# FalkorDB/FalkorDB

Hardware: NVIDIA B200
Metric: traversed edges/sec (mxm TEPS), 3-hop ANY_PAIR mxm chain (higher is better)
Workload: dtype bool/u32 index

## Files before the change

### falkordb_b200/csrc/bits.cu

```cuda
#include "common.cuh"
#include "ops.cuh"
#include <cub/block/block_reduce.cuh>
#include <algorithm>
#include <cstring>

namespace b200 {

template <int W> struct PullCfg {
    static constexpr int WL = W >= 4 ? 4 : W;
    static constexpr int SPLIT = W / WL;
    static constexpr int VG = 8 / SPLIT;
};
static const u64 PUSH_CHUNK = 8192;
static const u64 LONG_ROW = 4096;
static const u64 LONG_CHUNK = 8192;

static void require_natural(const DevBits &X, const char *what);

u32 bits_words_for(u64 nrows) {
    if (nrows == 0) return 1;
    u64 w = (nrows + 63) / 64;
    if (w > 16) return 0;
    u32 p = 1;
    while (p < w) p <<= 1;
    return p;
}

__global__ void k_bits_scatter(const u64 *__restrict__ Ap, const u32 *__restrict__ Aj, u64 nrows, u64 nnz,
                               u64 *__restrict__ X, u32 W) {
    u64 q = (u64)blockIdx.x * blockDim.x + threadIdx.x;
    u64 stride = (u64)gridDim.x * blockDim.x;
    for (; q < nnz; q += stride) {
        u64 lo = 0, hi = nrows - 1;
        while (lo < hi) {
            u64 mid = (lo + hi + 1) >> 1;
            if (Ap[mid] <= q) lo = mid; else hi = mid - 1;
        }
        u32 col = Aj[q];
        atomicOr((unsigned long long *)&X[(u64)col * W + (lo >> 6)], 1ULL << (lo & 63));
    }
}

void bits_from_csr(const DevCSR &F, DevBits &X) {
    u32 W = bits_words_for(F.nrows);
    if (!W) throw GrbError(-8, "bit-frontier form needs <= 1024 rows");
    X.clear();
    X.nrows = F.nrows; X.ncols = F.ncols; X.W = W;
    X.w.alloc(F.ncols * W);
    X.w.zero();
    if (F.nnz)
        LAUNCH(k_bits_scatter, grid_for(F.nnz, 256, 1 << 16), 256, 0, F.p.ptr, F.j.ptr, F.nrows, F.nnz, X.w.ptr, W);
}

static const u32 TILE_V = 1024;
static const u32 TILE_THREADS = 512;

__device__ __forceinline__ u32 transpose32(u32 x, u32 lane) {
    u32 y;
    y = __shfl_xor_sync(0xffffffffu, x, 16);
    x = (lane & 16) ? ((x & 0xFFFF0000u) | ((y & 0xFFFF0000u) >> 16)) : ((x & 0x0000FFFFu) | ((y & 0x0000FFFFu) << 16));
    y = __shfl_xor_sync(0xffffffffu, x, 8);
    x = (lane & 8) ? ((x & 0xFF00FF00u) | ((y & 0xFF00FF00u) >> 8)) : ((x & 0x00FF00FFu) | ((y & 0x00FF00FFu) << 8));
    y = __shfl_xor_sync(0xffffffffu, x, 4);
    x = (lane & 4) ? ((x & 0xF0F0F0F0u) | ((y & 0xF0F0F0F0u) >> 4)) : ((x & 0x0F0F0F0Fu) | ((y & 0x0F0F0F0Fu) << 4));
    y = __shfl_xor_sync(0xffffffffu, x, 2);
    x = (lane & 2) ? ((x & 0xCCCCCCCCu) | ((y & 0xCCCCCCCCu) >> 2)) : ((x & 0x33333333u) | ((y & 0x33333333u) << 2));
    y = __shfl_xor_sync(0xffffffffu, x, 1);
    x = (lane & 1) ? ((x & 0xAAAAAAAAu) | ((y & 0xAAAAAAAAu) >> 1)) : ((x & 0x55555555u) | ((y & 0x55555555u) << 1));
    return x;
}

__global__ void __launch_bounds__(TILE_THREADS)
k_bits_count(const u64 *__restrict__ X, u64 n, u32 W, u64 ntiles, u32 *__restrict__ tc) {
    __shared__ u32 wc[TILE_THREADS / 32][64];
    const u32 tid = threadIdx.x, warp = tid >> 5, lane = tid & 31;
    u64 tile = blockIdx.x;
    u64 v0 = tile * TILE_V + (u64)warp * 64;
    for (u32 w = 0; w < W; w++) {
        u32 clo = 0, chi = 0;
#pragma unroll
        for (u32 g = 0; g < 2; g++) {
            u64 v = v0 + g * 32 + lane;
            u64 word = (v < n) ? X[v * W + w] : 0ULL;
            if (__ballot_sync(0xffffffffu, word != 0ULL)) {
                clo += __popc(transpose32((u32)word, lane));
                chi += __popc(transpose32((u32)(word >> 32), lane));
            }
        }
        wc[warp][lane] = clo;
        wc[warp][lane + 32] = chi;
        __syncthreads();
        if (tid < 64) {
            u32 s = 0;
#pragma unroll
            for (u32 q = 0; q < TILE_THREADS / 32; q++) s += wc[q][tid];
            tc[((u64)w * 64 + tid) * ntiles + tile] = s;
        }
        __syncthreads();
    }
}

__device__ __forceinline__ void csa(u64 &hi, u64 &lo, u64 a, u64 b, u64 c) {
    const u64 u = a ^ b;
    hi = (a & b) | (u & c);
    lo = u ^ c;
}
template <int WL> __device__ __forceinline__ void ld_part(u64 (&x)[WL], const u64 *p) {
    if constexpr (WL == 1) { x[0] = __ldg(p); }
    else if constexpr (WL == 2) { ulonglong2 v = __ldg(reinterpret_cast<const ulonglong2 *>(p)); x[0] = v.x; x[1] = v.y; }
    else { u64x4 v = ld_v4(p); x[0] = v.a; x[1] = v.b; x[2] = v.c; x[3] = v.d; }
}
template <int W>
__global__ void __launch_bounds__(128)
k_bits_count_csa(const u64 *__restrict__ X, u64 n, u64 ntiles, u32 *__restrict__ tc) {
    constexpr int WL = PullCfg<W>::WL, SPLIT = PullCfg<W>::SPLIT;
    const u32 lane = threadIdx.x & 31;
    const u64 wid = ((u64)blockIdx.x * blockDim.x + threadIdx.x) >> 5;
    const u64 tile = wid / SPLIT;
    const u32 h = (u32)(wid % SPLIT);
    if (tile >= ntiles) return;
    const u64 vbase = tile * TILE_V;
    u64 plane[6][WL];
    u64 pend[5][WL];
#pragma unroll
    for (int p = 0; p < 6; p++)
#pragma unroll
        for (int w = 0; w < WL; w++) plane[p][w] = 0;
#pragma unroll
    for (int i = 0; i < 16; i++) {
        u64 xa[WL], xb[WL];
        const u64 va = vbase + lane + 64 * (u64)i, vb_ = va + 32;
        if (va < n) ld_part<WL>(xa, X + va * W + h * WL); else { for (int w = 0; w < WL; w++) xa[w] = 0; }
        if (vb_ < n) ld_part<WL>(xb, X + vb_ * W + h * WL); else { for (int w = 0; w < WL; w++) xb[w] = 0; }
#pragma unroll
        for (int w = 0; w < WL; w++) {
            u64 c;
            csa(c, plane[0][w], plane[0][w], xa[w], xb[w]);
#pragma unroll
            for (int L = 1; L < 6; L++) {
                if ((i >> (L - 1)) & 1) {
                    if (L < 5) { u64 c2; csa(c2, plane[L][w], plane[L][w], pend[L - 1][w], c); c = c2; }
                    else plane[5][w] ^= 0;
                } else { pend[L - 1][w] = c; break; }
            }
            if (i == 15) plane[5][w] = c;
        }
    }
#pragma unroll
    for (int w = 0; w < WL; w++) {
        u32 clo = 0, chi = 0;
#pragma unroll
        for (int p = 0; p < 6; p++) {
            clo += __popc(transpose32((u32)plane[p][w], lane)) << p;
            chi += __popc(transpose32((u32)(plane[p][w] >> 32), lane)) << p;
        }
        const u64 col = (u64)(h * WL + w) * 64;
        tc[(col + lane) * ntiles + tile] = clo;
        tc[(col + 32 + lane) * ntiles + tile] = chi;
    }
}

static const u32 FILL2_TSTRIDE = 33;
static const u32 FILL2_LIST = TILE_V + 4;
static const size_t FILL2_SMEM = 2 * 64 * FILL2_TSTRIDE * sizeof(u32) + (TILE_THREADS / 32) * FILL2_LIST * sizeof(unsigned short);
__global__ void __launch_bounds__(TILE_THREADS)
k_bits_fill_rows(const u64 *__restrict__ X, u64 n, u32 W, u64 ntiles, const u64 *__restrict__ off, u32 *__restrict__ Cj) {
    extern __shared__ __align__(16) unsigned char fill2_smem[];
    u32 *T = reinterpret_cast<u32 *>(fill2_smem);
    const u32 tid = threadIdx.x, warp = tid >> 5, lane = tid & 31;
    unsigned short *L = reinterpret_cast<unsigned short *>(fill2_smem + 2 * 64 * FILL2_TSTRIDE * sizeof(u32)) + warp * FILL2_LIST;
    const u32 NW = TILE_THREADS / 32;
    const u64 strm = policy_stream();
    const u64 tile = blockIdx.x;
    const u64 vbase = tile * TILE_V;
    const u32 vb = (u32)vbase;
    for (u32 w = 0; w < W; w++) {
        u32 *Tw = T + (w & 1) * 64 * FILL2_TSTRIDE;
#pragma unroll
        for (u32 g = 0; g < 2; g++) {
            u64 v = vbase + (u64)warp * 64 + g * 32 + lane;
            u64 word = (v < n) ? X[v * W + w] : 0ULL;
            u32 tl = 0, th = 0;
            if (__ballot_sync(0xffffffffu, word != 0ULL)) {
                tl = transpose32((u32)word, lane);
                th = transpose32((u32)(word >> 32), lane);
            }
            Tw[lane * FILL2_TSTRIDE + 2 * warp + g] = tl;
            Tw[(lane + 32) * FILL2_TSTRIDE + 2 * warp + g] = th;
        }
        __syncthreads();
        for (u32 r = warp; r < 64; r += NW) {
            u32 m = Tw[r * FILL2_TSTRIDE + lane];
            u32 c = __popc(m), incl = c;
#pragma unroll
            for (u32 d = 1; d < 32; d <<= 1) { u32 t = __shfl_up_sync(0xffffffffu, incl, d); if (lane >= d) incl += t; }
            const u32 cnt = __shfl_sync(0xffffffffu, incl, 31);
            if (cnt == 0) continue;
            const u64 g0 = off[((u64)w * 64 + r) * ntiles + tile];
            const u32 a = (u32)(g0 & 3);
            u32 o = a + incl - c;
            const u32 idb = lane * 32;
            while (m) { u32 bit = __ffs(m) - 1; L[o++] = (unsigned short)(idb + bit); m &= m - 1; }
            __syncwarp();
            u32 *dst = Cj + (g0 - a);
            const u32 total = a + cnt;
            const u32 head_end = a ? (total < 4 ? total : 4) : 0;
            if (lane >= a && lane < head_end) st_u32_stream(dst + lane, vb + L[lane], strm);
            const u32 nfull = total >> 2;
            const uint2 *L2 = reinterpret_cast<const uint2 *>(L);
            uint4 *dv = reinterpret_cast<uint4 *>(dst);
            for (u32 i = (a ? 1 : 0) + lane; i < nfull; i += 32) {
                uint2 p = L2[i];
                uint4 q;
                q.x = vb + (p.x & 0xFFFFu); q.y = vb + (p.x >> 16); q.z = vb + (p.y & 0xFFFFu); q.w = vb + (p.y >> 16);
                __stcs(dv + i, q);
            }
            const u32 tail = nfull * 4 > head_end ? nfull * 4 : head_end;
            if (tail + lane < total) st_u32_stream(dst + tail + lane, vb + L[tail + lane], strm);
            __syncwarp();
        }
    }
}

static const u32 F3_TILE = 2048, F3_THREADS = 512, F3_STRIDE = 66, F3_LIST = F3_TILE + 8;
static const size_t F3_SMEM = 2 * 64 * F3_STRIDE * sizeof(u32) + (F3_THREADS / 32) * F3_LIST * sizeof(unsigned short);
__global__ void __launch_bounds__(F3_THREADS, 2)
k_bits_fill_v3(const u64 *__restrict__ X, u64 n, u32 W, u64 ntiles1k, const u64 *__restrict__ off, u32 *__restrict__ Cj) {
    extern __shared__ __align__(16) unsigned char f3_smem[];
    u32 *T = reinterpret_cast<u32 *>(f3_smem);
    const u32 tid = threadIdx.x, warp = tid >> 5, lane = tid & 31;
    unsigned short *L = reinterpret_cast<unsigned short *>(f3_smem + 2 * 64 * F3_STRIDE * sizeof(u32)) + warp * F3_LIST;
    constexpr u32 NW = F3_THREADS / 32, RPW = 64 / NW;
    const u64 strm = policy_stream();
    const u64 tile = blockIdx.x;
    const u64 vbase = tile * F3_TILE;
    const u32 lo16base = (u32)(vbase & 0xFFFFu), vbhi = (u32)(vbase >> 16);
    for (u32 w = 0; w < W; w++) {
        u32 *Tw = T + (w & 1) * 64 * F3_STRIDE;
        u64 g0[RPW];
#pragma unroll
        for (u32 i = 0; i < RPW; i++) g0[i] = off[((u64)w * 64 + warp + NW * i) * ntiles1k + 2 * tile];
#pragma unroll
        for (u32 g = 0; g < 4; g++) {
            const u64 v = vbase + (u64)warp * 128 + g * 32 + lane;
            const u64 word = (v < n) ? X[v * W + w] : 0ULL;
            u32 tl = 0, th = 0;
            if (__ballot_sync(0xffffffffu, word != 0ULL)) {
                tl = transpose32((u32)word, lane);
                th = transpose32((u32)(word >> 32), lane);
            }
            Tw[lane * F3_STRIDE + 4 * warp + g] = tl;
            Tw[(lane + 32) * F3_STRIDE + 4 * warp + g] = th;
        }
        __syncthreads();
        u64 m[RPW];
        u32 c[RPW];
#pragma unroll
        for (u32 i = 0; i < RPW; i++) {
            m[i] = *reinterpret_cast<const u64 *>(Tw + (warp + NW * i) * F3_STRIDE + 2 * lane);
            c[i] = __popcll(m[i]);
        }
        u32 pk[RPW / 2];
#pragma unroll
        for (u32 h = 0; h < RPW / 2; h++) pk[h] = c[2 * h] | (c[2 * h + 1] << 16);
#pragma unroll
        for (u32 d = 1; d < 32; d <<= 1) {
#pragma unroll
            for (u32 h = 0; h < RPW / 2; h++) { const u32 t = __shfl_up_sync(0xffffffffu, pk[h], d); if (lane >= d) pk[h] += t; }
        }
#pragma unroll
        for (u32 i = 0; i < RPW; i++) {
            const u32 field = (i & 1) ? (pk[i / 2] >> 16) : (pk[i / 2] & 0xFFFFu);
            const u32 cnt = __shfl_sync(0xffffffffu, field, 31);
            if (cnt == 0) continue;
            const u32 a = (u32)(g0[i] & 3);
            u32 o = a + field - c[i];
            u32 idb = lo16base + lane * 64;
            u32 lo = (u32)m[i], hi = (u32)(m[i] >> 32);
            while (lo) { const u32 bit = __ffs(lo) - 1; L[o++] = (unsigned short)(idb + bit); lo &= lo - 1; }
            idb += 32;
            while (hi) { const u32 bit = __ffs(hi) - 1; L[o++] = (unsigned short)(idb + bit); hi &= hi - 1; }
            __syncwarp();
            u32 *dst = Cj + (g0[i] - a);
            const u32 total = a + cnt;
            const u32 head_end = a ? (total < 4 ? total : 4) : 0;
            if (lane >= a && lane < head_end) st_u32_stream(dst + lane, (vbhi << 16) | L[lane], strm);
            const u32 nfull = total >> 2;
            const uint2 *L2 = reinterpret_cast<const uint2 *>(L);
            uint4 *dv = reinterpret_cast<uint4 *>(dst);
            for (u32 k = (a ? 1 : 0) + lane; k < nfull; k += 32) {
                const uint2 p = L2[k];
                uint4 q;
                q.x = __byte_perm(p.x, vbhi, 0x5410); q.y = __byte_perm(p.x, vbhi, 0x5432);
                q.z = __byte_perm(p.y, vbhi, 0x5410); q.w = __byte_perm(p.y, vbhi, 0x5432);
                __stcs(dv + k, q);
            }
            const u32 tail = nfull * 4 > head_end ? nfull * 4 : head_end;
            if (tail + lane < total) st_u32_stream(dst + tail + lane, (vbhi << 16) | L[tail + lane], strm);
            __syncwarp();
        }
    }
}

__global__ void __launch_bounds__(TILE_THREADS)
k_bits_count_keep(const u64 *__restrict__ X, u64 n, u32 W, u64 ntiles, u32 *__restrict__ tc, u32 *__restrict__ Tg) {
    __shared__ __align__(16) u32 T[64 * FILL2_TSTRIDE];
    const u32 tid = threadIdx.x, warp = tid >> 5, lane = tid & 31;
    const u64 tile = blockIdx.x;
    const u64 vbase = tile * TILE_V;
    for (u32 w = 0; w < W; w++) {
#pragma unroll
        for (u32 g = 0; g < 2; g++) {
            u64 v = vbase + (u64)warp * 64 + g * 32 + lane;
            u64 word = (v < n) ? X[v * W + w] : 0ULL;
            u32 tl = 0, th = 0;
            if (__ballot_sync(0xffffffffu, word != 0ULL)) {
                tl = transpose32((u32)word, lane);
                th = transpose32((u32)(word >> 32), lane);
            }
            T[lane * FILL2_TSTRIDE + 2 * warp + g] = tl;
            T[(lane + 32) * FILL2_TSTRIDE + 2 * warp + g] = th;
        }
        __syncthreads();
        {
            const u32 r = tid >> 3, c4 = (tid & 7) * 4;
            uint4 q;
            q.x = T[r * FILL2_TSTRIDE + c4]; q.y = T[r * FILL2_TSTRIDE + c4 + 1];
            q.z = T[r * FILL2_TSTRIDE + c4 + 2]; q.w = T[r * FILL2_TSTRIDE + c4 + 3];
            u32 c = __popc(q.x) + __popc(q.y) + __popc(q.z) + __popc(q.w);
            c += __shfl_xor_sync(0xffffffffu, c, 1);
            c += __shfl_xor_sync(0xffffffffu, c, 2);
            c += __shfl_xor_sync(0xffffffffu, c, 4);
            if ((tid & 7) == 0) tc[((u64)w * 64 + r) * ntiles + tile] = c;
            *reinterpret_cast<uint4 *>(Tg + (((u64)w * ntiles + tile) * 64 + r) * 32 + c4) = q;
        }
        __syncthreads();
    }
}

static const u32 FILLM_WARPS = 8;
__global__ void __launch_bounds__(FILLM_WARPS * 32)
k_bits_fill_masks(const u32 *__restrict__ Tg, u32 W, u64 ntiles, const u64 *__restrict__ off, u32 *__restrict__ Cj) {
    __shared__ __align__(16) unsigned short lists[FILLM_WARPS][FILL2_LIST];
    const u32 warp = threadIdx.x >> 5, lane = threadIdx.x & 31;
    unsigned short *L = lists[warp];
    const u64 strm = policy_stream();
    const u64 ntasks = (u64)W * ntiles * 64;
    const u64 nwarps = (u64)gridDim.x * FILLM_WARPS;
    u64 task = (u64)blockIdx.x * FILLM_WARPS + warp;
    u32 mnext = task < ntasks ? __ldg(Tg + task * 32 + lane) : 0;
    for (; task < ntasks; task += nwarps) {
        u32 m = mnext;
        if (task + nwarps < ntasks) mnext = __ldg(Tg + (task + nwarps) * 32 + lane);
        u32 c = __popc(m), incl = c;
#pragma unroll
        for (u32 d = 1; d < 32; d <<= 1) { u32 t = __shfl_up_sync(0xffffffffu, incl, d); if (lane >= d) incl += t; }
        const u32 cnt = __shfl_sync(0xffffffffu, incl, 31);
        if (cnt == 0) continue;
        const u32 r = (u32)(task & 63);
        const u64 wt = task >> 6, w = wt / ntiles, tile = wt - w * ntiles;
        const u32 vb = (u32)(tile * TILE_V);
        const u64 g0 = off[(w * 64 + r) * ntiles + tile];
        const u32 a = (u32)(g0 & 3);
        u32 o = a + incl - c;
        const u32 idb = lane * 32;
        while (m) { u32 bit = __ffs(m) - 1; L[o++] = (unsigned short)(idb + bit); m &= m - 1; }
        __syncwarp();
        u32 *dst = Cj + (g0 - a);
        const u32 total = a + cnt;
        const u32 head_end = a ? (total < 4 ? total : 4) : 0;
        if (lane >= a && lane < head_end) st_u32_stream(dst + lane, vb + L[lane], strm);
        const u32 nfull = total >> 2;
        const uint2 *L2 = reinterpret_cast<const uint2 *>(L);
        uint4 *dv = reinterpret_cast<uint4 *>(dst);
        for (u32 i = (a ? 1 : 0) + lane; i < nfull; i += 32) {
            uint2 p = L2[i];
            uint4 q;
            q.x = vb + (p.x & 0xFFFFu); q.y = vb + (p.x >> 16); q.z = vb + (p.y & 0xFFFFu); q.w = vb + (p.y >> 16);
            __stcs(dv + i, q);
        }
        const u32 tail = nfull * 4 > head_end ? nfull * 4 : head_end;
        if (tail + lane < total) st_u32_stream(dst + tail + lane, vb + L[tail + lane], strm);
        __syncwarp();
    }
}

__global__ void __launch_bounds__(TILE_THREADS)
k_bits_fill(const u64 *__restrict__ X, u64 n, u32 W, u64 ntiles, const u64 *__restrict__ off, u32 *__restrict__ Cj,
            u32 cap) {
    extern __shared__ unsigned short list[];
    __shared__ unsigned short wp[TILE_THREADS / 32][64];
    __shared__ u32 sbase[65];
    __shared__ u64 goff[64];
    const u32 tid = threadIdx.x, warp = tid >> 5, lane = tid & 31;
    const u32 NW = TILE_THREADS / 32;
    const u64 strm = policy_stream();
    u64 tile = blockIdx.x;
    u64 vbase = tile * TILE_V;
    for (u32 w = 0; w < W; w++) {
        u32 tlo[2], thi[2];
        u32 clo = 0, chi = 0;
#pragma unroll
        for (u32 g = 0; g < 2; g++) {
            u64 v = vbase + (u64)warp * 64 + g * 32 + lane;
            u64 word = (v < n) ? X[v * W + w] : 0ULL;
            tlo[g] = 0; thi[g] = 0;
            if (__ballot_sync(0xffffffffu, word != 0ULL)) {
                tlo[g] = transpose32((u32)word, lane);
                thi[g] = transpose32((u32)(word >> 32), lane);
            }
            clo += __popc(tlo[g]);
            chi += __popc(thi[g]);
        }
        wp[warp][lane] = (unsigned short)clo;
        wp[warp][lane + 32] = (unsigned short)chi;
        __syncthreads();
        if (tid < 64) {
            u32 run = 0;
#pragma unroll
            for (u32 q = 0; q < NW; q++) { u32 t = wp[q][tid]; wp[q][tid] = (unsigned short)run; run += t; }
            sbase[tid + 1] = run;
            goff[tid] = off[((u64)w * 64 + tid) * ntiles + tile];
        }
        __syncthreads();
        if (tid == 0) {
            u32 run = 0;
            sbase[0] = 0;
            for (u32 r = 0; r < 64; r++) { u32 t = sbase[r + 1]; sbase[r + 1] = run + t; run += t; }
        }
        __syncthreads();
        const bool staged = sbase[64] <= cap;
        if (!staged) {
            u64 o = goff[lane] + wp[warp][lane];
#pragma unroll
            for (u32 g = 0; g < 2; g++) {
                u32 m = tlo[g];
                u64 idb = vbase + warp * 64 + g * 32;
                while (m) { u32 bit = __ffs(m) - 1; Cj[o++] = (u32)(idb + bit); m &= m - 1; }
            }
            o = goff[lane + 32] + wp[warp][lane + 32];
#pragma unroll
            for (u32 g = 0; g < 2; g++) {
                u32 m = thi[g];
                u64 idb = vbase + warp * 64 + g * 32;
                while (m) { u32 bit = __ffs(m) - 1; Cj[o++] = (u32)(idb + bit); m &= m - 1; }
            }
            __syncthreads();
            continue;
        }
        {
            u32 o = sbase[lane] + wp[warp][lane];
#pragma unroll
            for (u32 g = 0; g < 2; g++) {
                u32 m = tlo[g];
                u32 idb = warp * 64 + g * 32;
                while (m) { u32 bit = __ffs(m) - 1; list[o++] = (unsigned short)(idb + bit); m &= m - 1; }
            }
            o = sbase[lane + 32] + wp[warp][lane + 32];
#pragma unroll
            for (u32 g = 0; g < 2; g++) {
                u32 m = thi[g];
                u32 idb = warp * 64 + g * 32;
                while (m) { u32 bit = __ffs(m) - 1; list[o++] = (unsigned short)(idb + bit); m &= m - 1; }
            }
        }
        __syncthreads();
        for (u32 r = warp; r < 64; r += NW) {
            u32 s = sbase[r], cnt = sbase[r + 1] - s;
            u32 *dst = Cj + goff[r];
            for (u32 i = lane; i < cnt; i += 32) st_u32_stream(dst + i, (u32)(vbase + list[s + i]), strm);
        }
        __syncthreads();
    }
}

__global__ void k_bits_rowptr(const u64 *__restrict__ off, u64 nrows, u64 ntiles, u64 *__restrict__ Cp) {
    u64 r = (u64)blockIdx.x * blockDim.x + threadIdx.x;
    if (r <= nrows) Cp[r] = off[r * ntiles];
}

void bits_to_csr(const DevBits &X, DevCSR &C) {
    require_natural(X, "bits_to_csr");
    u64 n = X.ncols;
    u32 W = X.W;
    C.clear();
    C.nrows = X.nrows; C.ncols = n;
    C.p.alloc(X.nrows + 1);
    if (n == 0) { C.p.zero(); C.nnz = 0; return; }
    u64 ntiles = (n + TILE_V - 1) / TILE_V;
    u64 ncnt = (u64)64 * W * ntiles;
    DevBuf<u32> tc(ncnt + 1);
    DevBuf<u64> off(ncnt + 1);
    const bool keep_masks = ctx().opt_fill_kernel == 2 && ctx().opt_fill_cap <= 0;
    DevBuf<u32> masks;
    if (keep_masks) masks.alloc((u64)W * ntiles * 64 * 32);
    {
        TimedScope ts(TK_BITS_COUNT, 8ULL * W * n + (keep_masks ? 8ULL * W * ntiles * TILE_V : 0));
        if (keep_masks) LAUNCH(k_bits_count_keep, (u32)ntiles, TILE_THREADS, 0, X.w.ptr, n, W, ntiles, tc.ptr, masks.ptr);
        else if (ctx().opt_count_kernel == 1) {
            const u64 nwarps = ntiles * (W >= 4 ? W / 4 : 1);
            const u32 g = (u32)((nwarps + 3) / 4);
            switch (W) {
            case 1: LAUNCH((k_bits_count_csa<1>), g, 128, 0, X.w.ptr, n, ntiles, tc.ptr); break;
            case 2: LAUNCH((k_bits_count_csa<2>), g, 128, 0, X.w.ptr, n, ntiles, tc.ptr); break;
            case 4: LAUNCH((k_bits_count_csa<4>), g, 128, 0, X.w.ptr, n, ntiles, tc.ptr); break;
            case 8: LAUNCH((k_bits_count_csa<8>), g, 128, 0, X.w.ptr, n, ntiles, tc.ptr); break;
            default: LAUNCH((k_bits_count_csa<16>), g, 128, 0, X.w.ptr, n, ntiles, tc.ptr); break;
            }
        }
        else LAUNCH(k_bits_count, (u32)ntiles, TILE_THREADS, 0, X.w.ptr, n, W, ntiles, tc.ptr);
    }
    CUDA_TRY(cudaMemsetAsync(tc.ptr + ncnt, 0, sizeof(u32), stream()));
    exclusive_scan_u32_to_u64(tc.ptr, off.ptr, ncnt + 1);
    LAUNCH(k_bits_rowptr, grid_for(X.nrows + 1, 256), 256, 0, off.ptr, X.nrows, ntiles, C.p.ptr);
    u64 nnz = read_scalar(off.ptr + X.nrows * ntiles);
    C.nnz = nnz;
    C.j.alloc(nnz);
    if (nnz) {
        static bool attr_set = false;
        if (!attr_set) {
            CUDA_TRY(cudaFuncSetAttribute(k_bits_fill, cudaFuncAttributeMaxDynamicSharedMemorySize, (int)(64 * TILE_V * sizeof(unsigned short))));
            CUDA_TRY(cudaFuncSetAttribute(k_bits_fill_rows, cudaFuncAttributeMaxDynamicSharedMemorySize, (int)FILL2_SMEM));
            CUDA_TRY(cudaFuncSetAttribute(k_bits_fill_v3, cudaFuncAttributeMaxDynamicSharedMemorySize, (int)F3_SMEM));
            attr_set = true;
        }
        TimedScope ts(TK_BITS_FILL, 8ULL * W * n + 4 * nnz);
        if (keep_masks) {
            LAUNCH(k_bits_fill_masks, (u32)ctx().num_sms * 8, FILLM_WARPS * 32, 0, masks.ptr, W, ntiles, off.ptr, C.j.ptr);
        } else if (ctx().opt_fill_kernel == 3 && ctx().opt_fill_cap <= 0 && W <= 8) {
            LAUNCH(k_bits_fill_v3, (u32)((n + F3_TILE - 1) / F3_TILE), F3_THREADS, F3_SMEM, X.w.ptr, n, W, ntiles, off.ptr, C.j.ptr);
        } else if ((ctx().opt_fill_kernel == 1 || ctx().opt_fill_kernel == 3) && ctx().opt_fill_cap <= 0) {
            LAUNCH(k_bits_fill_rows, (u32)ntiles, TILE_THREADS, FILL2_SMEM, X.w.ptr, n, W, ntiles, off.ptr, C.j.ptr);
        } else {
            u64 avg = nnz / (ntiles * W) + 1;
            u32 cap = 8192;
            while (cap < 65536 && (u64)cap < avg + avg / 2) cap += 8192;
            if (ctx().opt_fill_cap > 0) cap = (u32)ctx().opt_fill_cap;
            const size_t smem = (size_t)cap * sizeof(unsigned short);
            LAUNCH(k_bits_fill, (u32)ntiles, TILE_THREADS, smem, X.w.ptr, n, W, ntiles, off.ptr, C.j.ptr, cap);
        }
    }
}

__global__ void __launch_bounds__(256) k_is_diagonal(const u64 *__restrict__ p, const u32 *__restrict__ j, u64 n, u32 *__restrict__ bad) {
    u64 r = (u64)blockIdx.x * blockDim.x + threadIdx.x;
    u64 stride = (u64)gridDim.x * blockDim.x;
    bool b = false;
    for (; r < n; r += stride) {
        u64 s = p[r], e = p[r + 1];
        if (e - s > 1 || (e - s == 1 && j[s] != (u32)r)) b = true;
    }
    if (__any_sync(0xffffffffu, b) && (threadIdx.x & 31) == 0) atomicOr(bad, 1u);
}
bool csr_is_diagonal(const DevCSR &A) {
    if (A.nrows != A.ncols || A.nnz > A.nrows) return false;
    if (A.nrows == 0) return true;
    DevBuf<u32> bad(1);
    bad.zero();
    LAUNCH(k_is_diagonal, grid_for(A.nrows, 256, 148 * 16), 256, 0, A.p.ptr, A.j.ptr, A.nrows, bad.ptr);
    return read_scalar(bad.ptr) == 0;
}
__global__ void __launch_bounds__(256)
k_bits_diag(const u64 *__restrict__ X, const u64 *__restrict__ Ap, u64 n, u32 W, u64 *__restrict__ Y, u64 *__restrict__ flops) {
    typedef cub::BlockReduce<u64, 256> Red;
    __shared__ typename Red::TempStorage ts;
    u64 t = (u64)blockIdx.x * blockDim.x + threadIdx.x;
    const u64 stride = (u64)gridDim.x * blockDim.x, total = n * W;
    u64 c = 0;
    for (; t < total; t += stride) {
        const u64 v = t / W;
        const u64 x = (Ap[v + 1] > Ap[v]) ? X[t] : 0ULL;
        Y[t] = x;
        c += __popcll(x);
    }
    u64 tot = Red(ts).Sum(c);
    if (threadIdx.x == 0 && tot) atomicAdd((unsigned long long *)flops, tot);
}
void bits_diag(const DevBits &X, const DevCSR &A, DevBits &Y, u64 *flops_out) {
    require_natural(X, "bits_diag");
    if (X.ncols != A.nrows) throw GrbError(-6, "mxm: inner dimensions differ");
    Y.clear();
    Y.nrows = X.nrows; Y.ncols = A.ncols; Y.W = X.W;
    Y.w.alloc(A.ncols * X.W);
    DevBuf<u64> fl(1);
    fl.zero();
    if (A.nrows) LAUNCH(k_bits_diag, grid_for(A.nrows * X.W, 256, 148 * 16), 256, 0, X.w.ptr, A.p.ptr, A.nrows, X.W, Y.w.ptr, fl.ptr);
    if (flops_out) *flops_out = read_scalar(fl.ptr);
}

__global__ void __launch_bounds__(TILE_THREADS)
k_bits_rowmajor(const u64 *__restrict__ X, u64 n, u32 W, u64 nrows, u64 wpr, u64 *__restrict__ out) {
    __shared__ u32 T[2][64 * FILL2_TSTRIDE];
    const u32 tid = threadIdx.x, warp = tid >> 5, lane = tid & 31;
    const u64 tile = blockIdx.x;
    const u64 vbase = tile * TILE_V;
    const u64 strm = policy_stream();
    for (u32 w = 0; w < W; w++) {
        if ((u64)w * 64 >= nrows) break;
        u32 *Tw = T[w & 1];
#pragma unroll
        for (u32 g = 0; g < 2; g++) {
            u64 v = vbase + (u64)warp * 64 + g * 32 + lane;
            u64 word = (v < n) ? X[v * W + w] : 0ULL;
            u32 tl = 0, th = 0;
            if (__ballot_sync(0xffffffffu, word != 0ULL)) {
                tl = transpose32((u32)word, lane);
                th = transpose32((u32)(word >> 32), lane);
            }
            Tw[lane * FILL2_TSTRIDE + 2 * warp + g] = tl;
            Tw[(lane + 32) * FILL2_TSTRIDE + 2 * warp + g] = th;
        }
        __syncthreads();
#pragma unroll
        for (u32 h = 0; h < 2; h++) {
            u32 r = (tid >> 4) + 32 * h, c = tid & 15;
            u64 row = (u64)w * 64 + r, col = tile * (TILE_V / 64) + c;
            if (row < nrows && col < wpr) {
                u64 val = (u64)Tw[r * FILL2_TSTRIDE + 2 * c] | ((u64)Tw[r * FILL2_TSTRIDE + 2 * c + 1] << 32);
                st_u64_stream(out + row * wpr + col, val, strm);
            }
        }
    }
}

void bits_to_rowmajor(const DevBits &X, u64 *out, u64 wpr) {
    require_natural(X, "bits_to_rowmajor");
    u64 n = X.ncols;
    if (!n || !X.nrows) return;
    u64 ntiles = (n + TILE_V - 1) / TILE_V;
    LAUNCH(k_bits_rowmajor, (u32)ntiles, TILE_THREADS, 0, X.w.ptr, n, X.W, X.nrows, wpr, out);
}

__global__ void k_csr_to_bitmap(const u64 *__restrict__ p, const u32 *__restrict__ j, u64 nrows, u64 wpr, u64 *__restrict__ out) {
    u64 row = ((u64)blockIdx.x * blockDim.x + threadIdx.x) >> 5;
    u32 lane = threadIdx.x & 31;
    if (row >= nrows) return;
    for (u64 q = p[row] + lane; q < p[row + 1]; q += 32) {
        u32 c = j[q];
        atomicOr((unsigned long long *)(out + row * wpr + (c >> 6)), 1ULL << (c & 63));
    }
}
void csr_to_rowmajor(const DevCSR &A, u64 *out, u64 wpr) {
    if (!A.nrows || !A.nnz) return;
    LAUNCH(k_csr_to_bitmap, grid_for(A.nrows * 32, 256), 256, 0, A.p.ptr, A.j.ptr, A.nrows, wpr, out);
}

__global__ void __launch_bounds__(256) k_popc_sum(const u64 *__restrict__ w, u64 n, u64 *__restrict__ out) {
    typedef cub::BlockReduce<u64, 256> Red;
    __shared__ typename Red::TempStorage ts;
    u64 t = (u64)blockIdx.x * blockDim.x + threadIdx.x;
    u64 stride = (u64)gridDim.x * blockDim.x;
    u64 s = 0;
    for (; t < n; t += stride) s += __popcll(w[t]);
    u64 tot = Red(ts).Sum(s);
    if (threadIdx.x == 0 && tot) atomicAdd((unsigned long long *)out, tot);
}

u64 bits_nvals(const DevBits &X) {
    DevBuf<u64> out(1);
    out.zero();
    u64 n = X.ncols * X.W;
    if (n) LAUNCH(k_popc_sum, grid_for(n, 256, 148 * 8), 256, 0, X.w.ptr, n, out.ptr);
    return read_scalar(out.ptr);
}

__global__ void __launch_bounds__(256)
k_bits_flops(const u64 *__restrict__ X, u32 W, u64 n, const u64 *__restrict__ Ap, u32 *__restrict__ flag,
             u64 *__restrict__ out ) {
    typedef cub::BlockReduce<u64, 256> Red;
    __shared__ typename Red::TempStorage ts, ts2;
    u64 k = (u64)blockIdx.x * blockDim.x + threadIdx.x;
    u64 stride = (u64)gridDim.x * blockDim.x;
    u64 fl = 0, ed = 0;
    for (; k < n; k += stride) {
        u32 pc = 0;
        for (u32 w = 0; w < W; w++) pc += __popcll(X[k * W + w]);
        u64 d = Ap[k + 1] - Ap[k];
        flag[k] = (pc != 0 && d != 0) ? 1u : 0u;
        if (pc) { fl += (u64)pc * d; ed += d; }
    }
    u64 tf = Red(ts).Sum(fl);
    u64 te = Red(ts2).Sum(ed);
    if (threadIdx.x == 0) {
        if (tf) atomicAdd((unsigned long long *)&out[0], tf);
        if (te) atomicAdd((unsigned long long *)&out[1], te);
    }
}

__global__ void k_compact_active(const u32 *__restrict__ flag, const u64 *__restrict__ pos, u64 n,
                                 const u64 *__restrict__ Ap, u32 *__restrict__ act, u64 *__restrict__ deg,
                                 u64 *__restrict__ astart) {
    u64 k = (u64)blockIdx.x * blockDim.x + threadIdx.x;
    u64 stride = (u64)gridDim.x * blockDim.x;
    for (; k < n; k += stride) {
        if (flag[k]) {
            u64 d = pos[k];
            act[d] = (u32)k;
            u64 s = Ap[k];
            deg[d] = Ap[k + 1] - s;
            astart[d] = s;
        }
    }
}

__device__ __forceinline__ u64 find_le64(const u64 *__restrict__ a, u64 lo, u64 hi, u64 target) {
    while (lo < hi) {
        u64 mid = (lo + hi + 1) >> 1;
        if (a[mid] <= target) lo = mid; else hi = mid - 1;
    }
    return lo;
}

template <int W>
__global__ void __launch_bounds__(256)
k_bits_push(const u32 *__restrict__ act, const u64 *__restrict__ cum, const u64 *__restrict__ astart, u64 nact,
            u64 total, const u32 *__restrict__ Aj, const u64 *__restrict__ X, u64 *__restrict__ Y) {
    __shared__ u64 s_e0, s_e1;
    const u32 tid = threadIdx.x, warp = tid >> 5, lane = tid & 31;
    u64 lo = (u64)blockIdx.x * PUSH_CHUNK, hi = lo + PUSH_CHUNK;
    if (hi > total) hi = total;
    if (tid == 0) {
        s_e0 = find_le64(cum, 0, nact - 1, lo);
        s_e1 = find_le64(cum, 0, nact - 1, hi - 1);
    }
    __syncthreads();
    u64 e0 = s_e0, e1 = s_e1;
    for (u64 t0 = lo + (u64)warp * 32; t0 < hi; t0 += 8 * 32) {
        u64 e = find_le64(cum, e0, e1, t0);
        u64 t = t0 + lane;
        if (t < hi) {
            while (e < e1 && cum[e + 1] <= t) e++;
            u32 k = act[e];
            u32 col = Aj[astart[e] + (t - cum[e])];
#pragma unroll
            for (int w = 0; w < W; w++) {
                u64 xw = X[(u64)k * W + w];
                if (xw) atomicOr((unsigned long long *)&Y[(u64)col * W + w], xw);
            }
        }
    }
}

__global__ void k_csr_entry_info(const u64 *__restrict__ Fp, const u32 *__restrict__ Fj, u64 nrows, const u64 *__restrict__ Ap,
                                 u32 *__restrict__ erow, u64 *__restrict__ edeg) {
    u64 warp = ((u64)blockIdx.x * blockDim.x + threadIdx.x) >> 5;
    u32 lane = threadIdx.x & 31;
    if (warp >= nrows) return;
    for (u64 q = Fp[warp] + lane; q < Fp[warp + 1]; q += 32) {
        u32 k = Fj[q];
        erow[q] = (u32)warp;
        edeg[q] = Ap[k + 1] - Ap[k];
    }
}
template <int W>
__global__ void __launch_bounds__(256)
k_csr_push(const u32 *__restrict__ erow, const u32 *__restrict__ Fj, const u64 *__restrict__ cum, u64 nent, u64 total,
           const u64 *__restrict__ Ap, const u32 *__restrict__ Aj, u64 *__restrict__ Y, const u32 *__restrict__ perm) {
    __shared__ u64 s_e0, s_e1;
    const u32 tid = threadIdx.x, warp = tid >> 5, lane = tid & 31;
    u64 lo = (u64)blockIdx.x * PUSH_CHUNK, hi = lo + PUSH_CHUNK;
    if (hi > total) hi = total;
    if (tid == 0) {
        s_e0 = find_le64(cum, 0, nent - 1, lo);
        s_e1 = find_le64(cum, 0, nent - 1, hi - 1);
    }
    __syncthreads();
    u64 e0 = s_e0, e1 = s_e1;
    for (u64 t0 = lo + (u64)warp * 32; t0 < hi; t0 += 8 * 32) {
        u64 e = find_le64(cum, e0, e1, t0);
        u64 t = t0 + lane;
        if (t < hi) {
            while (e < e1 && cum[e + 1] <= t) e++;
            const u32 i = erow[e];
            u32 col = Aj[Ap[Fj[e]] + (t - cum[e])];
            if (perm) col = __ldg(perm + col);
            atomicOr((unsigned long long *)&Y[(u64)col * W + (i >> 6)], 1ULL << (i & 63));
        }
    }
}
template <int W>
static void csr_push_impl(const DevCSR &F, const DevCSR &A, DevBits &Y, u64 flops, const u32 *erow, const u64 *cum, const u32 *perm) {
    u64 nchunks = (flops + PUSH_CHUNK - 1) / PUSH_CHUNK;
    TimedScope ts(TK_BITS_PUSH, 4 * flops + 16 * F.nnz + 8 * flops);
    LAUNCH((k_csr_push<W>), (u32)nchunks, 256, 0, erow, F.j.ptr, cum, F.nnz, flops, A.p.ptr, A.j.ptr, Y.w.ptr, perm);
}
bool bits_push_from_csr(const DevCSR &F, const DevCSR &A, DevBits &Y, u64 *flops_out, const LongRows *lr) {
    if (F.ncols != A.nrows) throw GrbError(-6, "mxm: inner dimensions differ");
    const u32 W = bits_words_for(F.nrows);
    u64 flops = 0;
    DevBuf<u32> erow(F.nnz);
    DevBuf<u64> cum(F.nnz + 1);
    if (F.nnz) {
        LAUNCH(k_csr_entry_info, grid_for(F.nrows * 32, 256), 256, 0, F.p.ptr, F.j.ptr, F.nrows, A.p.ptr, erow.ptr, cum.ptr);
        CUDA_TRY(cudaMemsetAsync(cum.ptr + F.nnz, 0, sizeof(u64), stream()));
        exclusive_scan_u64(cum.ptr, cum.ptr, F.nnz + 1);
        flops = read_scalar(cum.ptr + F.nnz);
    }
    if (flops * 4 > A.nnz) return false;
    Y.clear();
    Y.nrows = F.nrows; Y.ncols = A.ncols; Y.W = W;
    Y.w.alloc(A.ncols * W);
    Y.w.zero();
    if (flops_out) *flops_out = flops;
    const u32 *perm = nullptr;
    if (lr && ctx().opt_perm_push && lr->perm_tag && lr->pperm && A.nrows == A.ncols && lr->pperm->n == A.ncols) {
        perm = lr->pperm->ptr;
        Y.pvert = lr->pvert;
        Y.perm_tag = lr->perm_tag;
    }
    if (flops == 0) return true;
    switch (W) {
    case 1: csr_push_impl<1>(F, A, Y, flops, erow.ptr, cum.ptr, perm); break;
    case 2: csr_push_impl<2>(F, A, Y, flops, erow.ptr, cum.ptr, perm); break;
    case 4: csr_push_impl<4>(F, A, Y, flops, erow.ptr, cum.ptr, perm); break;
    case 8: csr_push_impl<8>(F, A, Y, flops, erow.ptr, cum.ptr, perm); break;
    default: csr_push_impl<16>(F, A, Y, flops, erow.ptr, cum.ptr, perm); break;
    }
    return true;
}

__global__ void k_unpermute(const u64 *__restrict__ X, const u32 *__restrict__ pvert, u64 n, u32 W, u64 *__restrict__ out) {
    u64 t = (u64)blockIdx.x * blockDim.x + threadIdx.x;
    const u64 stride = (u64)gridDim.x * blockDim.x, total = n * W;
    for (; t < total; t += stride) { const u64 s = t / W, w = t - s * W; out[(u64)pvert[s] * W + w] = X[t]; }
}
void bits_naturalise(DevBits &X) {
    if (!X.permuted()) return;
    const u64 n = X.ncols;
    DevBuf<u64> out(n * X.W);
    if (n) LAUNCH(k_unpermute, grid_for(n * X.W, 256, 148 * 32), 256, 0, X.w.ptr, X.pvert->ptr, n, X.W, out.ptr);
    X.w = std::move(out);
    X.pvert.reset();
    X.perm_tag = 0;
}
// ... 1421 lines not shown
```

Before: 3137 billion.

## Replace fill_v3 with W-templated per-tile fill kernel loading all words upfront

Replaces the 2048-vertex fill kernel with a kernel templated on word count W that loads all of a tile's X words with vectorized loads and transposes every row into shared memory. Per-row offsets and counts are staged in shared memory, so all-zero rows are skipped without reading mask bits. Rows are processed two at a time with a packed shuffle scan, and set bits are written in descending order using bfind. This covers W up to 16 and aims to cut the per-word syncs and strided loads, in exchange for higher shared memory use and register pressure at large W.

```diff
diff --git a/falkordb_b200/csrc/bits.cu b/falkordb_b200/csrc/bits.cu
--- a/falkordb_b200/csrc/bits.cu
+++ b/falkordb_b200/csrc/bits.cu
@@ -222,72 +222,100 @@
     }
 }
 
-static const u32 F3_TILE = 2048, F3_THREADS = 512, F3_STRIDE = 66, F3_LIST = F3_TILE + 8;
-static const size_t F3_SMEM = 2 * 64 * F3_STRIDE * sizeof(u32) + (F3_THREADS / 32) * F3_LIST * sizeof(unsigned short);
-__global__ void __launch_bounds__(F3_THREADS, 2)
-k_bits_fill_v3(const u64 *__restrict__ X, u64 n, u32 W, u64 ntiles1k, const u64 *__restrict__ off, u32 *__restrict__ Cj) {
-    extern __shared__ __align__(16) unsigned char f3_smem[];
-    u32 *T = reinterpret_cast<u32 *>(f3_smem);
+static const u32 FT_THREADS = 512, FT_STRIDE = 33, FT_LIST = TILE_V + 8;
+static size_t fill_tile_smem(u32 W) {
+    return (size_t)64 * W * (sizeof(u64) + FT_STRIDE * sizeof(u32) + sizeof(u32)) + (FT_THREADS / 32) * FT_LIST * sizeof(unsigned short);
+}
+template <int W>
+__global__ void __launch_bounds__(FT_THREADS, W <= 8 ? 2 : 1)
+k_bits_fill_tile(const u64 *__restrict__ X, u64 n, u64 ntiles, const u32 *__restrict__ tc, const u64 *__restrict__ off,
+                 u32 *__restrict__ Cj) {
+    constexpr int WL = PullCfg<W>::WL;
+    constexpr u32 R = 64 * W;
+    extern __shared__ __align__(16) unsigned char ft_smem[];
     const u32 tid = threadIdx.x, warp = tid >> 5, lane = tid & 31;
-    unsigned short *L = reinterpret_cast<unsigned short *>(f3_smem + 2 * 64 * F3_STRIDE * sizeof(u32)) + warp * F3_LIST;
-    constexpr u32 NW = F3_THREADS / 32, RPW = 64 / NW;
+    u64 *goff = reinterpret_cast<u64 *>(ft_smem);
+    u32 *T = reinterpret_cast<u32 *>(goff + R);
+    u32 *cnt = T + R * FT_STRIDE;
+    unsigned short *L = reinterpret_cast<unsigned short *>(cnt + R) + warp * FT_LIST;
+    const u64 tile = blockIdx.x;
+    const u64 vbase = tile * TILE_V;
+    for (u32 i = tid; i < R; i += FT_THREADS) {
+        const u64 idx = (u64)i * ntiles + tile;
+        goff[i] = off[idx];
+        cnt[i] = tc[idx];
+    }
+    u64 x[2][W];
+#pragma unroll
+    for (u32 g = 0; g < 2; g++) {
+        const u64 v = vbase + (u64)warp * 64 + g * 32 + lane;
+#pragma unroll
+        for (int h = 0; h < W / WL; h++) {
+            u64 t[WL];
+            if (v < n) ld_part<WL>(t, X + v * W + h * WL);
+            else {
+#pragma unroll
+                for (int q = 0; q < WL; q++) t[q] = 0;
+            }
+#pragma unroll
+            for (int q = 0; q < WL; q++) x[g][h * WL + q] = t[q];
+        }
+    }
+#pragma unroll
+    for (int w = 0; w < W; w++) {
+#pragma unroll
+        for (u32 g = 0; g < 2; g++) {
+            u32 tl = 0, th = 0;
+            if (__ballot_sync(0xffffffffu, x[g][w] != 0ULL)) {
+                tl = transpose32((u32)x[g][w], lane);
+                th = transpose32((u32)(x[g][w] >> 32), lane);
+            }
+            T[(w * 64 + lane) * FT_STRIDE + 2 * warp + g] = tl;
+            T[(w * 64 + 32 + lane) * FT_STRIDE + 2 * warp + g] = th;
+        }
+    }
+    __syncthreads();
     const u64 strm = policy_stream();
-    const u64 tile = blockIdx.x;
-    const u64 vbase = tile * F3_TILE;
-    const u32 lo16base = (u32)(vbase & 0xFFFFu), vbhi = (u32)(vbase >> 16);
-    for (u32 w = 0; w < W; w++) {
-        u32 *Tw = T + (w & 1) * 64 * F3_STRIDE;
-        u64 g0[RPW];
-#pragma unroll
-        for (u32 i = 0; i < RPW; i++) g0[i] = off[((u64)w * 64 + warp + NW * i) * ntiles1k + 2 * tile];
-#pragma unroll
-        for (u32 g = 0; g < 4; g++) {
-            const u64 v = vbase + (u64)warp * 128 + g * 32 + lane;
-            const u64 word = (v < n) ? X[v * W + w] : 0ULL;
-            u32 tl = 0, th = 0;
-            if (__ballot_sync(0xffffffffu, word != 0ULL)) {
-                tl = transpose32((u32)word, lane);
-                th = transpose32((u32)(word >> 32), lane);
-            }
-            Tw[lane * F3_STRIDE + 4 * warp + g] = tl;
-            Tw[(lane + 32) * F3_STRIDE + 4 * warp + g] = th;
-        }
-        __syncthreads();
-        u64 m[RPW];
-        u32 c[RPW];
-#pragma unroll
-        for (u32 i = 0; i < RPW; i++) {
-            m[i] = *reinterpret_cast<const u64 *>(Tw + (warp + NW * i) * F3_STRIDE + 2 * lane);
-            c[i] = __popcll(m[i]);
-        }
-        u32 pk[RPW / 2];
-#pragma unroll
-        for (u32 h = 0; h < RPW / 2; h++) pk[h] = c[2 * h] | (c[2 * h + 1] << 16);
-#pragma unroll
-        for (u32 d = 1; d < 32; d <<= 1) {
-#pragma unroll
-            for (u32 h = 0; h < RPW / 2; h++) { const u32 t = __shfl_up_sync(0xffffffffu, pk[h], d); if (lane >= d) pk[h] += t; }
-        }
-#pragma unroll
-        for (u32 i = 0; i < RPW; i++) {
-            const u32 field = (i & 1) ? (pk[i / 2] >> 16) : (pk[i / 2] & 0xFFFFu);
-            const u32 cnt = __shfl_sync(0xffffffffu, field, 31);
-            if (cnt == 0) continue;
-            const u32 a = (u32)(g0[i] & 3);
-            u32 o = a + field - c[i];
-            u32 idb = lo16base + lane * 64;
-            u32 lo = (u32)m[i], hi = (u32)(m[i] >> 32);
-            while (lo) { const u32 bit = __ffs(lo) - 1; L[o++] = (unsigned short)(idb + bit); lo &= lo - 1; }
-            idb += 32;
-            while (hi) { const u32 bit = __ffs(hi) - 1; L[o++] = (unsigned short)(idb + bit); hi &= hi - 1; }
+    const u32 vbhi = (u32)(vbase >> 16);
+    const u32 idb = (u32)(vbase & 0xFFFFu) + lane * 32;
+#pragma unroll 1
+    for (u32 r0 = warp; r0 < R; r0 += 2 * FT_THREADS / 32) {
+        const u32 r1 = r0 + FT_THREADS / 32;
+        const u32 tot0 = cnt[r0], tot1 = cnt[r1];
+        if ((tot0 | tot1) == 0) continue;
+        const u32 m0 = T[r0 * FT_STRIDE + lane], m1 = T[r1 * FT_STRIDE + lane];
+        const u32 c = __popc(m0) | (__popc(m1) << 16);
+        u32 incl = c;
+#pragma unroll
+        for (u32 d = 1; d < 32; d <<= 1) { const u32 t = __shfl_up_sync(0xffffffffu, incl, d); if (lane >= d) incl += t; }
+#pragma unroll
+        for (u32 h = 0; h < 2; h++) {
+            const u32 total = h ? tot1 : tot0;
+            if (total == 0) continue;
+            const u64 g0 = goff[h ? r1 : r0];
+            const u32 a = (u32)(g0 & 3);
+            unsigned short *e = L + a + (h ? (incl >> 16) : (incl & 0xFFFFu));
+            u32 mm = h ? m1 : m0;
+            while (mm) {
+                u32 b;
+                asm("bfind.u32 %0, %1;" : "=r"(b) : "r"(mm));
+                mm ^= 1u << b;
+                e[-1] = (unsigned short)(idb + b);
+                if (!mm) break;
+                asm("bfind.u32 %0, %1;" : "=r"(b) : "r"(mm));
+                mm ^= 1u << b;
+                e[-2] = (unsigned short)(idb + b);
+                e -= 2;
+            }
             __syncwarp();
-            u32 *dst = Cj + (g0[i] - a);
-            const u32 total = a + cnt;
-            const u32 head_end = a ? (total < 4 ? total : 4) : 0;
+            u32 *dst = Cj + (g0 - a);
+            const u32 end = a + total;
+            const u32 head_end = a ? (end < 4 ? end : 4) : 0;
             if (lane >= a && lane < head_end) st_u32_stream(dst + lane, (vbhi << 16) | L[lane], strm);
-            const u32 nfull = total >> 2;
+            const u32 nfull = end >> 2;
             const uint2 *L2 = reinterpret_cast<const uint2 *>(L);
             uint4 *dv = reinterpret_cast<uint4 *>(dst);
+#pragma unroll 1
             for (u32 k = (a ? 1 : 0) + lane; k < nfull; k += 32) {
                 const uint2 p = L2[k];
                 uint4 q;
@@ -296,10 +324,21 @@
                 __stcs(dv + k, q);
             }
             const u32 tail = nfull * 4 > head_end ? nfull * 4 : head_end;
-            if (tail + lane < total) st_u32_stream(dst + tail + lane, (vbhi << 16) | L[tail + lane], strm);
+            if (tail + lane < end) st_u32_stream(dst + tail + lane, (vbhi << 16) | L[tail + lane], strm);
             __syncwarp();
         }
     }
+}
+
+template <int W>
+static void fill_tile(const u64 *X, u64 n, u64 ntiles, const u32 *tc, const u64 *off, u32 *Cj) {
+    const size_t smem = fill_tile_smem(W);
+    static bool attr_set = false;
+    if (!attr_set) {
+        CUDA_TRY(cudaFuncSetAttribute(k_bits_fill_tile<W>, cudaFuncAttributeMaxDynamicSharedMemorySize, (int)smem));
+        attr_set = true;
+    }
+    LAUNCH((k_bits_fill_tile<W>), (u32)ntiles, FT_THREADS, smem, X, n, ntiles, tc, off, Cj);
 }
 
 __global__ void __launch_bounds__(TILE_THREADS)
@@ -521,15 +560,20 @@
         if (!attr_set) {
             CUDA_TRY(cudaFuncSetAttribute(k_bits_fill, cudaFuncAttributeMaxDynamicSharedMemorySize, (int)(64 * TILE_V * sizeof(unsigned short))));
             CUDA_TRY(cudaFuncSetAttribute(k_bits_fill_rows, cudaFuncAttributeMaxDynamicSharedMemorySize, (int)FILL2_SMEM));
-            CUDA_TRY(cudaFuncSetAttribute(k_bits_fill_v3, cudaFuncAttributeMaxDynamicSharedMemorySize, (int)F3_SMEM));
             attr_set = true;
         }
         TimedScope ts(TK_BITS_FILL, 8ULL * W * n + 4 * nnz);
         if (keep_masks) {
             LAUNCH(k_bits_fill_masks, (u32)ctx().num_sms * 8, FILLM_WARPS * 32, 0, masks.ptr, W, ntiles, off.ptr, C.j.ptr);
-        } else if (ctx().opt_fill_kernel == 3 && ctx().opt_fill_cap <= 0 && W <= 8) {
-            LAUNCH(k_bits_fill_v3, (u32)((n + F3_TILE - 1) / F3_TILE), F3_THREADS, F3_SMEM, X.w.ptr, n, W, ntiles, off.ptr, C.j.ptr);
-        } else if ((ctx().opt_fill_kernel == 1 || ctx().opt_fill_kernel == 3) && ctx().opt_fill_cap <= 0) {
+        } else if (ctx().opt_fill_kernel == 3 && ctx().opt_fill_cap <= 0) {
+            switch (W) {
+            case 1: fill_tile<1>(X.w.ptr, n, ntiles, tc.ptr, off.ptr, C.j.ptr); break;
+            case 2: fill_tile<2>(X.w.ptr, n, ntiles, tc.ptr, off.ptr, C.j.ptr); break;
+            case 4: fill_tile<4>(X.w.ptr, n, ntiles, tc.ptr, off.ptr, C.j.ptr); break;
+            case 8: fill_tile<8>(X.w.ptr, n, ntiles, tc.ptr, off.ptr, C.j.ptr); break;
+            default: fill_tile<16>(X.w.ptr, n, ntiles, tc.ptr, off.ptr, C.j.ptr); break;
+            }
+        } else if (ctx().opt_fill_kernel == 1 && ctx().opt_fill_cap <= 0) {
             LAUNCH(k_bits_fill_rows, (u32)ntiles, TILE_THREADS, FILL2_SMEM, X.w.ptr, n, W, ntiles, off.ptr, C.j.ptr);
         } else {
             u64 avg = nnz / (ntiles * W) + 1;
```

Measured after the change: 3204 billion (median of 6 runs). 1.02x the previous value.
